# csukuangfj/kaldi-hmm-gmm

Measured on AMD Instinct MI355X. Metric: frames/sec (whole node) per EM iter (align+acc-stats), 5k-pdf x 64-Gauss, higher is better.
Workload: dtype f32 via f16x2s

## Files before the change

kaldi_hmm_gmm_amd/csrc/khg_k3.hip:

```cpp
#include "khg_internal.hpp"

#include <hipcub/hipcub.hpp>

#include "khg_k3_accstats.hip.inc"
#include "khg_k3_post.hip.inc"
#include "khg_k3_accops.hip.inc"

extern "C" int khg_accs_create(khg_ctx* ctx, const khg_model* m, const khg_tm* tm, khg_accs** out) {
  if (ctx_dead(ctx) || !m || !tm || !out) return khg_set_error(KHG_E_ARG, "khg_accs_create: bad arguments");
  khg_accs* a = new khg_accs();
  a->ctx = ctx; a->sumG = m->sumG; a->D = m->D; a->num_tids = tm->num_tids;
  a->n = a->sumG * (1 + 2 * (int64_t)a->D) + a->num_tids + 1 + 8;
  int rc = dev_alloc(&a->buf_d, (size_t)a->n);
  if (rc) { delete a; return rc; }
  a->cap = a->n;
  *out = a;
  return khg_accs_zero(ctx, a);
}
extern "C" int khg_accs_destroy(khg_accs* a) { if (a) { DEVFREE(a->buf_d); DEVFREE(a->wire_d); delete a; } return KHG_OK; }
extern "C" int khg_accs_zero(khg_ctx* ctx, khg_accs* a) {
  if (ctx_dead(ctx) || !a) return khg_set_error(KHG_E_ARG, "bad arguments");
  HIPCHK(hipMemsetAsync(a->buf_d, 0, sizeof(double) * (size_t)a->n, ctx->stream));
  return KHG_OK;
}
// ... 211 lines not shown
          KHG_LAUNCH(ctx, k3_sub_scan, dim3(1), dim3(1024), 0, ctx->stream, u->unc_d, u->frame_off_d, u->n_utt, u->sub_off_d);
          KHG_LAUNCH(ctx, k3_sub_keys, dim3((unsigned)std::min(u->n_utt, 8192)), dim3(64), 0, ctx->stream, a, u->unc_d, u->frame_off_d, u->sub_off_d, u->n_utt, sort_keys, sort_vals);
        } else if (tm->num_tids <= K3_LDS_TIDS) KHG_LAUNCH(ctx, k3_sort_keys<true>, dim3(std::min(gb, 1024)), dim3(256), 0, ctx->stream, a, sort_keys, sort_vals);
        else KHG_LAUNCH(ctx, k3_sort_keys<false>, dim3(std::min(gb, 1024)), dim3(256), 0, ctx->stream, a, sort_keys, sort_vals);
        HIPCHK(hipcub::DeviceRadixSort::SortPairs(sort_tmp, need, sort_keys, sort_keys_out, sort_vals,
                                                  reinterpret_cast<uint32_t*>(a.frame_ids), (int)Neff, 0, bits, ctx->stream));
        if (post) {
          K3Args b = a;
          b.num_tids = -1;
          KHG_LAUNCH(ctx, k3_bounds, dim3((m->P + 256) / 256), dim3(256), 0, ctx->stream, b, sort_keys_out);
        } else KHG_LAUNCH(ctx, k3_bounds, dim3((m->P + 256) / 256), dim3(256), 0, ctx->stream, a, sort_keys_out);
      }
    }
    int64_t k3_extra_blocks = 0;
    auto make_items = [&](int ny_base, bool parked, size_t nsum1, int cls_lo, int cls_hi, bool second) -> int {
      const int64_t avg = Neff / std::max(1, m->P);
      const int target = ctx->k3_one_block ? INT_MAX : (int)std::min<int64_t>(1 << 30, std::max<int64_t>(512, 2 * avg / ny_base));
      const int64_t per_t = Neff / target;
      k3_extra_blocks = std::min<int64_t>(per_t + m->P, 2 * per_t) + 1;
      const int64_t max_items = (int64_t)m->P * ny_base + k3_extra_blocks;
      const int64_t max_slots = !parked ? INT_MAX : ny_base > 1 ? max_items : 2 * per_t + 1;
      if (max_items >= INT_MAX / 2) return khg_set_error(KHG_E_UNSUPPORTED, "khg_acc_stats: too many work items");
      if (u->k3_items_n < (size_t)max_items) {
        DEVFREE(u->k3_items_d);
        { int ri = u_alloc(u, reinterpret_cast<K3Item**>(&u->k3_items_d), 2 * (size_t)max_items); if (ri) return ri; }
        u->k3_items_n = (size_t)max_items;
      }
      if (u->k3_item_off_n < (size_t)m->P + 1) {
        DEVFREE(u->k3_item_off_d);
        int rc2 = u_alloc(u, &u->k3_item_off_d, 2 * ((size_t)m->P + 1));
        if (rc2) return rc2;
        u->k3_item_off_n = (size_t)m->P + 1;
      }
      if (parked && u->k3_part_n < (size_t)max_slots * nsum1) {
        DEVFREE(u->k3_part_d);
        int rc2 = u_alloc(u, &u->k3_part_d, (size_t)max_slots * nsum1);
        if (rc2) return rc2;
        u->k3_part_n = (size_t)max_slots * nsum1;
      }
      K3Item* items = reinterpret_cast<K3Item*>(u->k3_items_d) + (second ? u->k3_items_n : 0);
      int32_t* item_off = u->k3_item_off_d + (second ? u->k3_item_off_n : 0);
      KHG_LAUNCH(ctx, k3_make_items, dim3(1), dim3(1024), 0, ctx->stream, a, ny_base, target, (int)max_items, (int)std::min<int64_t>(max_slots, INT_MAX),
                         items, item_off, cls_lo, cls_hi);
      a.items = items; a.item_off = item_off;
      return KHG_OK;
    };
    const int k3form = ctx->opt[KHG_OPT_K3_FORM];
    auto run_wave = [&](int cls_lo, int cls_hi, int maxG, void* comm_) -> int {
      const int nb = (maxG + 15) / 16;
      bool f16a = false;
      if (nb >= 3 && ctx->opt[KHG_OPT_K3_PHASE_A] == 0 && ctx->opt[KHG_OPT_K3_PHASE_B] != 1) { rc = k3_phase_a_scales(ctx, const_cast<khg_model*>(m), u, &f16a); if (rc) return rc; }
      if (f16a) {
        a.pa_ex = m->k3_ex_d; a.pa_S = m->k3_S;
        a.pa_scale = std::ldexp(1.0f, m->k3_S); a.pa_inv = std::ldexp(1.0f, -m->k3_S); a.pa_c1 = std::ldexp(1.44269504088896340736f, -m->k3_S);
      }
      const bool f16b = f16a && ctx->opt[KHG_OPT_K3_PHASE_B] == 2 && std::isfinite(weight) && std::fabs(weight) > 1.0e-30f && std::fabs(weight) < 1.0e30f;
      if (f16b) { a.pb_SG = 13 - std::ilogb(std::fabs(weight)); a.pb_gscale = std::ldexp(1.0f, a.pb_SG); }
      const size_t lds = std::max<size_t>(f16a ? sizeof(float) * (4 * 4 * 16 * 20) + 2 * (size_t)(4 * 2 * 16 * K3_XH_ROW)
                                               : sizeof(float) * ((size_t)nb * 20 * 64 + 4 * 4 * 16 * 20),
                                          sizeof(double) * ((size_t)nb * 16 * 80 + (size_t)nb * 16));
      const int64_t avg_tiles = (Neff / std::max(1, m->P) + 15) / 16;
      int ny = (int)std::max<int64_t>(1, std::min<int64_t>(std::min<int64_t>(32, (avg_tiles + 15) / 16), (4096 + m->P - 1) / m->P));
      if (ctx->opt[KHG_OPT_K3_NY] > 0) ny = ctx->opt[KHG_OPT_K3_NY];
      const size_t nsum1 = (size_t)nb * 16 * 80 + (size_t)nb * 16 + 1;
      if (u->k3_llpart_n < (size_t)m->P) {
        DEVFREE(u->k3_llpart_d);
        rc = u_alloc(u, &u->k3_llpart_d, (size_t)m->P);
        if (rc) return rc;
        u->k3_llpart_n = (size_t)m->P;
      }
      rc = make_items(ny, true, nsum1, cls_lo, cls_hi, false);
      if (rc) return rc;
      HIPCHK(hipMemsetAsync(u->k3_llpart_d, 0, sizeof(double) * (size_t)m->P, ctx->stream));
      a.ll_part = u->k3_llpart_d;
      a.part = u->k3_part_d;
      const int nparts_ = comm_ ? nparts : 1;
      for (int part = 0; part < nparts_; ++part) {
      const int p0 = (int)((int64_t)m->P * part / nparts_), np = (int)((int64_t)m->P * (part + 1) / nparts_) - p0;
      a.pdf0 = p0; a.npdf = np;
      const unsigned nblk = (unsigned)((int64_t)np * ny + k3_extra_blocks);
      {
      KernelTimer kt(ctx, nsub < 0 ? "k3_accumulate" : "k3_accumulate_pass2");
      const bool exact_b = true;
      const size_t lds16 = std::max<size_t>(2 * (size_t)4 * (2 * (2 * 16 * K3_XH_ROW) + 2 * 2 * 40 * 36) + (size_t)nb * 3 * 2 * 64 * 16,
                                            sizeof(double) * ((size_t)nb * 16 * 80 + (size_t)nb * 16));
#define K3_WAVE_LAUNCH(NBV)                                                                                            \
  do {                                                                                                                  \
    if (f16b) {                                                                                                          \
      HIPCHK(hipFuncSetAttribute((const void*)k3_accumulate_wave16<NBV>, hipFuncAttributeMaxDynamicSharedMemorySize, (int)lds16)); \
      KHG_LAUNCH(ctx, (k3_accumulate_wave16<NBV>), dim3(nblk), dim3(256), lds16, ctx->stream, a);                     \
    } else if (exact_b && f16a) KHG_LAUNCH(ctx, (k3_accumulate_wave<NBV, true>), dim3(nblk), dim3(256), lds, ctx->stream, a);    \
    else KHG_LAUNCH(ctx, (k3_accumulate_wave<NBV>), dim3(nblk), dim3(256), lds, ctx->stream, a);                      \
    KHG_LAUNCH(ctx, (k3_wave_finalize<NBV>), dim3(np), dim3(256), 0, ctx->stream, a);                                 \
  } while (0)
      switch (nb) {
        case 1: K3_WAVE_LAUNCH(1); break;
        case 2: K3_WAVE_LAUNCH(2); break;
        case 3: K3_WAVE_LAUNCH(3); break;
        default: K3_WAVE_LAUNCH(4); break;
      }
#undef K3_WAVE_LAUNCH
      }
      if (comm_ && nparts_ > 1) { rc = accs_allreduce_pieces(ctx, acc, m, p0, np, comm_, nullptr); if (rc) return rc; }
      }
      a.pdf0 = 0; a.npdf = m->P;
      KHG_LAUNCH(ctx, k3_wave_scalars, dim3(1), dim3(1024), 0, ctx->stream, a, cls_lo, cls_hi);
      return KHG_OK;
    };
    auto run_mfma = [&](int cls_lo, int cls_hi, int maxG, int n_cls, bool second, void* comm_) -> int {
      const int64_t avg_chunks = (Neff / std::max(1, m->P) + K3_CHUNK - 1) / K3_CHUNK;
      const size_t lds = sizeof(float) * ((size_t)4 * K3_CHUNK * 2 * m->KQ + (post ? 6 : 5) * K3_CHUNK);
      int ny = (int)std::max<int64_t>(1, std::min<int64_t>(std::min<int64_t>(32, avg_chunks), (4096 + n_cls - 1) / std::max(1, n_cls)));
      if (ctx->opt[KHG_OPT_K3_NY] > 0) ny = ctx->opt[KHG_OPT_K3_NY];
      if (ctx->k3_one_block) ny = 1;
      rc = make_items(ny, false, 0, cls_lo, cls_hi, second);
      if (rc) return rc;
      bool b16 = false;
      if (!post && ctx->opt[KHG_OPT_K3_PHASE_A] == 0 && ctx->opt[KHG_OPT_K3_PHASE_B] == 2 && ((m->KQ == 20 && maxG <= 128) || (m->KQ == 10 && maxG <= 192)) &&
          std::isfinite(weight) && std::fabs(weight) > 1.0e-30f && std::fabs(weight) < 1.0e30f) {
        rc = k3_phase_a_scales(ctx, const_cast<khg_model*>(m), u, &b16);
        if (rc) return rc;
      }
      if (b16) {
        a.pa_ex = m->k3_ex_d; a.pa_S = m->k3_S;
        a.pa_scale = std::ldexp(1.0f, m->k3_S); a.pa_inv = std::ldexp(1.0f, -m->k3_S); a.pa_c1 = std::ldexp(1.44269504088896340736f, -m->k3_S);
        a.pb_SG = 13 - std::ilogb(std::fabs(weight)); a.pb_gscale = std::ldexp(1.0f, a.pb_SG);
      }
      const size_t kpad = ((size_t)8 * m->KQ + 31) / 32 * 32;
      const size_t gp_b16 = maxG <= 64 ? 64 : (maxG <= 128 ? 128 : 192);
      const size_t lds_b16 = std::max<size_t>(2 * (2 * (size_t)K3_CHUNK * (kpad + 8) + 2 * (size_t)8 * m->KQ * (K3_CHUNK + 8)) + sizeof(float) * 9 * K3_CHUNK,
                                              sizeof(float) * (2 * gp_b16 * (size_t)(m->D | 1) + 8 * (size_t)m->KQ));
      const int nparts_ = comm_ ? nparts : 1;
      for (int part = 0; part < nparts_; ++part) {
        const int p0 = (int)((int64_t)m->P * part / nparts_), np = (int)((int64_t)m->P * (part + 1) / nparts_) - p0;
        a.pdf0 = p0; a.npdf = np;
        const unsigned nblk = (unsigned)((int64_t)std::min(np, n_cls) * ny + k3_extra_blocks);
        {
          KernelTimer kt(ctx, nsub < 0 ? "k3_accumulate" : "k3_accumulate_pass2");
          if (b16) {
#define K3_B16(KQV, NBWV, NWVV)                                                                                                 \
  do {                                                                                                                          \
    HIPCHK(hipFuncSetAttribute((const void*)k3_accumulate_block16<KQV, NBWV, NWVV>, hipFuncAttributeMaxDynamicSharedMemorySize, (int)lds_b16)); \
    KHG_LAUNCH(ctx, (k3_accumulate_block16<KQV, NBWV, NWVV>), dim3(nblk), dim3(64 * NWVV), lds_b16, ctx->stream, a);            \
  } while (0)
            if (maxG <= 64) { if (m->KQ == 20) K3_B16(20, 1, 4); else K3_B16(10, 1, 4); }
            else if (maxG <= 128) { if (m->KQ == 20) K3_B16(20, 1, 8); else K3_B16(10, 1, 8); }
            else K3_B16(10, 3, 4);
#undef K3_B16
          } else if (post) {
            if (m->KQ == 10 && maxG <= 64) KHG_LAUNCH(ctx, (k3_accumulate_mfma<10, 1, true>), dim3(nblk), dim3(256), lds, ctx->stream, a);
            else if (m->KQ == 10 && maxG <= 128) KHG_LAUNCH(ctx, (k3_accumulate_mfma<10, 2, true>), dim3(nblk), dim3(256), lds, ctx->stream, a);
            else if (m->KQ == 10 && maxG <= 192) KHG_LAUNCH(ctx, (k3_accumulate_mfma<10, 3, true>), dim3(nblk), dim3(256), lds, ctx->stream, a);
            else if (m->KQ == 10) KHG_LAUNCH(ctx, (k3_accumulate_mfma<10, 4, true>), dim3(nblk), dim3(256), lds, ctx->stream, a);
            else if (maxG <= 64) KHG_LAUNCH(ctx, (k3_accumulate_mfma<20, 1, true>), dim3(nblk), dim3(256), lds, ctx->stream, a);
            else KHG_LAUNCH(ctx, (k3_accumulate_mfma<20, 2, true>), dim3(nblk), dim3(256), lds, ctx->stream, a);
          } else
          if (m->KQ == 10 && maxG <= 64) KHG_LAUNCH(ctx, (k3_accumulate_mfma<10, 1>), dim3(nblk), dim3(256), lds, ctx->stream, a);
          else if (m->KQ == 10 && maxG <= 128) KHG_LAUNCH(ctx, (k3_accumulate_mfma<10, 2>), dim3(nblk), dim3(256), lds, ctx->stream, a);
          else if (m->KQ == 10 && maxG <= 192) KHG_LAUNCH(ctx, (k3_accumulate_mfma<10, 3>), dim3(nblk), dim3(256), lds, ctx->stream, a);
          else if (m->KQ == 10) KHG_LAUNCH(ctx, (k3_accumulate_mfma<10, 4>), dim3(nblk), dim3(256), lds, ctx->stream, a);
          else if (maxG <= 64) KHG_LAUNCH(ctx, (k3_accumulate_mfma<20, 1>), dim3(nblk), dim3(256), lds, ctx->stream, a);
          else KHG_LAUNCH(ctx, (k3_accumulate_mfma<20, 2>), dim3(nblk), dim3(256), lds, ctx->stream, a);
        }
        if (comm_ && nparts_ > 1) { rc = accs_allreduce_pieces(ctx, acc, m, p0, np, comm_, nullptr); if (rc) return rc; }
      }
      a.pdf0 = 0; a.npdf = m->P;
      return KHG_OK;
// ... 154 lines not shown
```

kaldi_hmm_gmm_amd/csrc/khg_k3_accstats.hip.inc:

```

struct K3Args {
  const float* feats;
  const int32_t* ali;
  const int32_t* id2pdf;
  int32_t num_tids;
  int64_t N;
  int32_t P, D;
  const int32_t* gauss_off;
  const float* gconsts;
  const float* means_invvars;
  const float* inv_vars;
  const float* nhalf_inv_vars;
  int32_t* pdf_count;
  int64_t* pdf_start;
  int32_t* pdf_cursor;
  int32_t* frame_ids;
  unsigned long long* tid_count;
  double* occ; double* mean_acc; double* var_acc; double* trans_acc; double* scalars;
  float weight;
  int32_t* err_flag;
  double* part;
  double* ll_part;
  int32_t pdf0, npdf;
  const struct K3Item* items;
// ... 797 lines not shown
          if (!(fabsf(llf) <= 3.0e38f)) atomicOr(a.err_flag, 1);
          tot_ll += (double)(llf * wf);
          if constexpr (POST) tot_w += (double)wf;
        }
        const float scale = f < cf ? wf / ssum : 0.0f;
#pragma unroll
        for (int k = 0; k < NBW; ++k) ll[k][ft][r] = ll[k][ft][r] * scale;
      }
#pragma unroll
    for (int ft = 0; ft < 4; ++ft) {
#pragma unroll
      for (int s = 0; s < 4; ++s) {
        const int fr = 16 * ft + 4 * q + s;
        double ga[NBW];
#pragma unroll
        for (int k = 0; k < NBW; ++k) { ga[k] = (double)ll[k][ft][s]; occ[k] += ga[k]; }
#pragma unroll
        for (int db = 0; db < NDB; ++db) {
          const int col = 16 * db + j16;
          const int d = col < XP ? col : col - XP;
          const double bv = (double)xq[(((col < XP ? 0 : 2) + (d & 1)) * K3_CHUNK + fr) * KH + (d >> 1)];
#pragma unroll
          for (int k = 0; k < NBW; ++k)
            acc[k][db] = __builtin_amdgcn_mfma_f64_16x16x4f64(ga[k], bv, acc[k][db], 0, 0, 0);
        }
      }
    }
  }
#pragma unroll
  for (int k = 0; k < NBW; ++k) {
    const int gb = 16 * (wave + 4 * k);
#pragma unroll
    for (int db = 0; db < NDB; ++db) {
      const int col = 16 * db + j16;
#pragma unroll
      for (int r = 0; r < 4; ++r) {
        const int g = gb + q + 4 * r;
        if (g < G) {
          if (col < D) atomicAdd(a.mean_acc + (int64_t)(g0 + g) * D + col, acc[k][db][r]);
          else if (col >= XP && col - XP < D) atomicAdd(a.var_acc + (int64_t)(g0 + g) * D + (col - XP), acc[k][db][r]);
        }
      }
    }
    double o = occ[k];
    o += __shfl_xor(o, 16);
    o += __shfl_xor(o, 32);
    if (q == 0 && gb + j16 < G) atomicAdd(a.occ + g0 + gb + j16, o);
  }
  if (wave == 0) {
    for (int o2 = 32; o2 > 0; o2 >>= 1) tot_ll += __shfl_xor(tot_ll, o2);
    if (lane == 0 && tot_ll != 0.0) atomicAdd(&a.scalars[1], tot_ll);
  }
  if constexpr (POST) {
    if (wave == 0) {
      for (int o2 = 32; o2 > 0; o2 >>= 1) tot_w += __shfl_xor(tot_w, o2);
      if (lane == 0 && tot_w != 0.0) atomicAdd(&a.scalars[0], tot_w);
    }
  } else {
    if (tid == 0 && it.y == 0) atomicAdd(&a.scalars[0], (double)nfr * (double)a.weight);
  }
}

typedef _Float16 k3_f16x8 __attribute__((ext_vector_type(8)));
#define K3_XH_ROW 104

template <int NB>
__device__ __forceinline__ void k3_wave_flush(const K3Args& a, const double* sum, int g0, int G, int D, int tid) {
  constexpr int XP = 40;
  for (int i = tid; i < NB * 16 * 2 * XP; i += 256) {
    const int g = i / (2 * XP), col = i - g * (2 * XP);
    if (g < G) {
      if (col < D) atomicAdd(a.mean_acc + (int64_t)(g0 + g) * D + col, sum[i]);
      else if (col >= XP && col - XP < D) atomicAdd(a.var_acc + (int64_t)(g0 + g) * D + (col - XP), sum[i]);
    }
  }
  if (tid < NB * 16 && tid < G) atomicAdd(a.occ + g0 + tid, sum[NB * 16 * 2 * XP + tid]);
}

__device__ __forceinline__ void k3_lds_sync() {
  asm volatile("s_waitcnt lgkmcnt(0)" ::: "memory");
  __builtin_amdgcn_wave_barrier();
}

template <int NB, bool F16A = false>
__global__ __launch_bounds__(256, NB <= 2 ? 2 : 1) void k3_accumulate_wave(K3Args a) {
  extern __shared__ __attribute__((aligned(16))) float k3s[];
  constexpr int KQ = 10, XP = 4 * KQ, KH = 2 * KQ, NDB = KQ / 2, TF = 16;
  K3Item it;
  if (!k3_take_item(a, it)) return;
  const int pdf = it.pdf;
  const int64_t beg = a.pdf_start[pdf];
  const int nfr = (int)(a.pdf_start[pdf + 1] - beg);
  if (nfr == 0) return;
  const int D = a.D;
  const int g0 = a.gauss_off[pdf], G = a.gauss_off[pdf + 1] - g0;
  const int tid = threadIdx.x, lane = tid & 63;
  const int wave = __builtin_amdgcn_readfirstlane(tid >> 6);
  const int j16 = lane & 15, q = lane >> 4;
  float* Wl = k3s;
  float* xw = (F16A ? k3s : Wl + NB * KH * 64) + wave * (4 * TF * KH);
  _Float16* xh = reinterpret_cast<_Float16*>(k3s + 4 * (4 * TF * KH)) + wave * (2 * TF * K3_XH_ROW);
  float gcv[NB];
#pragma unroll
  for (int k = 0; k < NB; ++k) gcv[k] = (16 * k + j16 < G) ? a.gconsts[g0 + 16 * k + j16] : -INFINITY;
  float wq[F16A ? 1 : NB][F16A ? 1 : KH];
  k3_f16x8 w1[F16A ? NB : 1][3], w2[F16A ? NB : 1][3];
  if constexpr (!F16A) {
    for (int idx = tid; idx < NB * KH * 64; idx += 256) {
      const int l = idx & 63, s = (idx >> 6) % KH, k = idx / (64 * KH);
      const int g = 16 * k + (l & 15), qq = l >> 4, d = 2 * s + (qq & 1);
      float v = 0.0f;
      if (g < G && d < D) v = (qq & 2) ? a.nhalf_inv_vars[(int64_t)(g0 + g) * D + d] : a.means_invvars[(int64_t)(g0 + g) * D + d];
      Wl[idx] = v;
    }
    __syncthreads();
#pragma unroll
    for (int k = 0; k < NB; ++k)
#pragma unroll
      for (int s = 0; s < KH; ++s) wq[k][s] = Wl[(k * KH + s) * 64 + lane];
  } else {
#pragma unroll
    for (int k = 0; k < NB; ++k)
#pragma unroll
      for (int st = 0; st < 3; ++st) {
        k3_f16x8 p1, p2;
#pragma unroll
        for (int e = 0; e < 8; ++e) {
          const int kp = 32 * st + 8 * q + e, var = kp >= XP, d = var ? kp - XP : kp, g = 16 * k + j16;
          float v = 0.0f;
          if (kp < 2 * XP && g < G && d < D) {
            const float w = var ? a.nhalf_inv_vars[(int64_t)(g0 + g) * D + d] : a.means_invvars[(int64_t)(g0 + g) * D + d];
            v = ldexpf(w, a.pa_S - a.pa_ex[2 * d + var]);
          }
          const _Float16 h1 = (_Float16)v;
          p1[e] = h1; p2[e] = (_Float16)(v - (float)h1);
        }
        w1[k][st] = p1; w2[k][st] = p2;
      }
#pragma unroll
    for (int k = 0; k < NB; ++k) gcv[k] = gcv[k] * a.pa_scale;
    for (int i = lane; i < 2 * TF * K3_XH_ROW; i += 64) xh[i] = (_Float16)0.0f;
    k3_lds_sync();
  }
  (void)Wl; (void)wq; (void)w1; (void)w2;

  f64x4 acc[NB][NDB];
  double occ[NB];
#pragma unroll
  for (int k = 0; k < NB; ++k) {
    occ[k] = 0.0;
#pragma unroll
    for (int db = 0; db < NDB; ++db) acc[k][db] = f64x4{0, 0, 0, 0};
  }
  double tot_ll = 0.0;
  const int ntile = (nfr + TF - 1) / TF;
  constexpr int NG = TF * XP / 64;
  const int tstride = 4 * it.ny;
  float pre[NG];
  float sx[F16A ? NG : 1], sx2[F16A ? NG : 1];
  if constexpr (F16A) {
#pragma unroll
    for (int j = 0; j < NG; ++j) {
      const int d = min((lane + 64 * j) % XP, D - 1);
      sx[j] = ldexpf(1.0f, a.pa_ex[2 * d]); sx2[j] = ldexpf(1.0f, a.pa_ex[2 * d + 1]);
    }
  }
// ... 70 lines not shown
      }
    }
#pragma unroll
    for (int r = 0; r < 4; ++r) {
      float m = ll[0][r];
#pragma unroll
      for (int k = 1; k < NB; ++k) m = fmaxf(m, ll[k][r]);
      m = k3_row_max(m);
      float ssum = 0.0f;
#pragma unroll
      for (int k = 0; k < NB; ++k) {
        const float e = __builtin_amdgcn_exp2f((ll[k][r] - m) * (F16A ? a.pa_c1 : 1.44269504088896340736f));
        ll[k][r] = e;
        ssum += e;
      }
      ssum = k3_row_sum(ssum);
      const int f = 4 * q + r;
      if (j16 == 0 && f < cf) {
        const float llf = __logf(ssum) + (F16A ? m * a.pa_inv : m);
        if (!(fabsf(llf) <= 3.0e38f)) atomicOr(a.err_flag, 1);
        tot_ll += (double)(llf * a.weight);
      }
      const float scale = f < cf ? a.weight / ssum : 0.0f;
#pragma unroll
      for (int k = 0; k < NB; ++k) ll[k][r] = ll[k][r] * scale;
    }
#pragma unroll
    for (int s = 0; s < 4; ++s) {
      const int fr = 4 * q + s;
      double ga[NB];
#pragma unroll
      for (int k = 0; k < NB; ++k) { ga[k] = (double)ll[k][s]; occ[k] += ga[k]; }
#pragma unroll
      for (int db = 0; db < NDB; ++db) {
        const int col = 16 * db + j16;
        const int d = col < XP ? col : col - XP;
        const double bv = (double)xw[(((col < XP ? 0 : 2) + (d & 1)) * TF + fr) * KH + (d >> 1)];
#pragma unroll
        for (int k = 0; k < NB; ++k)
          acc[k][db] = __builtin_amdgcn_mfma_f64_16x16x4f64(ga[k], bv, acc[k][db], 0, 0, 0);
      }
    }
    k3_lds_sync();
  }
  __syncthreads();
  double* sum = reinterpret_cast<double*>(k3s);
  constexpr int NSUM = NB * 16 * 2 * XP + NB * 16;
  for (int i = tid; i < NSUM; i += 256) sum[i] = 0.0;
  __syncthreads();
#pragma unroll 1
  for (int w = 0; w < 4; ++w) {
    if (wave == w) {
#pragma unroll
      for (int k = 0; k < NB; ++k) {
#pragma unroll
        for (int db = 0; db < NDB; ++db) {
          const int col = 16 * db + j16;
#pragma unroll
          for (int r = 0; r < 4; ++r) atomicAdd(&sum[(16 * k + q + 4 * r) * (2 * XP) + col], acc[k][db][r]);
        }
        double o = occ[k];
        o += __shfl_xor(o, 16);
        o += __shfl_xor(o, 32);
        if (q == 0) atomicAdd(&sum[NB * 16 * 2 * XP + 16 * k + j16], o);
      }
    }
    __syncthreads();
  }
  __shared__ double s_ll[4];
  for (int o2 = 32; o2 > 0; o2 >>= 1) tot_ll += __shfl_xor(tot_ll, o2);
  if (lane == 0) s_ll[wave] = tot_ll;
  __syncthreads();
  const double block_ll = ((s_ll[0] + s_ll[1]) + s_ll[2]) + s_ll[3];
  if (it.ny == 1) {
    k3_wave_flush<NB>(a, sum, g0, G, D, tid);
    if (tid == 0) a.ll_part[pdf] = block_ll;
  } else {
    double* dst = a.part + (int64_t)it.slot * (NSUM + 1);
    for (int i = tid; i < NSUM; i += 256) dst[i] = sum[i];
    if (tid == 0) dst[NSUM] = block_ll;
  }
}

template <int NB>
__global__ __launch_bounds__(256, 1) void k3_accumulate_wave16(K3Args a) {
  extern __shared__ __attribute__((aligned(16))) float k3s[];
  constexpr int KQ = 10, XP = 4 * KQ, NDB = KQ / 2, TF = 16;
  constexpr int XHH = 2 * TF * K3_XH_ROW;
  constexpr int XTR = 36, XTH = 2 * 2 * XP * XTR;
  K3Item it;
  if (!k3_take_item(a, it)) return;
  const int pdf = it.pdf;
  const int64_t beg = a.pdf_start[pdf];
  const int nfr = (int)(a.pdf_start[pdf + 1] - beg);
  if (nfr == 0) return;
  const int D = a.D;
  const int g0 = a.gauss_off[pdf], G = a.gauss_off[pdf + 1] - g0;
  const int tid = threadIdx.x, lane = tid & 63;
  const int wave = __builtin_amdgcn_readfirstlane(tid >> 6);
  const int j16 = lane & 15, q = lane >> 4;
  _Float16* xh = reinterpret_cast<_Float16*>(k3s) + wave * (2 * XHH + XTH);
  _Float16* xt = xh + 2 * XHH;
  float gcv[NB];
#pragma unroll
  for (int k = 0; k < NB; ++k) gcv[k] = ((16 * k + j16 < G) ? a.gconsts[g0 + 16 * k + j16] : -INFINITY) * a.pa_scale;
  char* wl16 = reinterpret_cast<char*>(reinterpret_cast<_Float16*>(k3s) + 4 * (2 * XHH + XTH));
  for (int e0 = tid; e0 < NB * 3 * 64; e0 += 256) {
    const int l = e0 & 63, st = (e0 >> 6) % 3, k = e0 / (3 * 64), jl = l & 15, ql = l >> 4;
    k3_f16x8 p1, p2;
#pragma unroll
    for (int e = 0; e < 8; ++e) {
      const int kp = 32 * st + 8 * ql + e, var = kp >= XP, d = var ? kp - XP : kp, g = 16 * k + jl;
      float v = 0.0f;
      if (kp < 2 * XP && g < G && d < D) {
        const float w = var ? a.nhalf_inv_vars[(int64_t)(g0 + g) * D + d] : a.means_invvars[(int64_t)(g0 + g) * D + d];
        v = ldexpf(w, a.pa_S - a.pa_ex[2 * d + var]);
      }
      const _Float16 h1 = (_Float16)v;
      p1[e] = h1; p2[e] = (_Float16)(v - (float)h1);
    }
    *reinterpret_cast<k3_f16x8*>(wl16 + (((k * 3 + st) * 2 + 0) * 64 + l) * 16) = p1;
    *reinterpret_cast<k3_f16x8*>(wl16 + (((k * 3 + st) * 2 + 1) * 64 + l) * 16) = p2;
  }
  {
    static_assert((2 * XHH + XTH) % 8 == 0, "the wave's planes are whole 16-byte words");
    const k3_f16x8 z = {0, 0, 0, 0, 0, 0, 0, 0};
    for (int i = lane; i < (2 * XHH + XTH) / 8; i += 64) reinterpret_cast<k3_f16x8*>(xh)[i] = z;
  }
  __syncthreads();

  f64x4 acc[NB][NDB];
  double occ[NB];
#pragma unroll
  for (int k = 0; k < NB; ++k) {
    occ[k] = 0.0;
#pragma unroll
    for (int db = 0; db < NDB; ++db) acc[k][db] = f64x4{0, 0, 0, 0};
  }
  double tot_ll = 0.0;
  unsigned bad = 0;
  const int ntile = (nfr + TF - 1) / TF, npair = (ntile + 1) / 2;
  constexpr int NM = 2 * TF * XP / (4 * 64);
  static_assert(NM * 4 * 64 == 2 * TF * XP, "micro-tiles cover the pair exactly");
  const int pstride = 4 * it.ny;
  float pre[NM][4];
  float sx[NM][2], sx2[NM][2];
  const bool even_d = (D & 1) == 0;
#pragma unroll
  for (int j = 0; j < NM; ++j)
#pragma unroll
    for (int c = 0; c < 2; ++c) {
      const int d = min(2 * ((lane + 64 * j) % 20) + c, D - 1);
      sx[j][c] = ldexpf(1.0f, a.pa_ex[2 * d]); sx2[j][c] = ldexpf(1.0f, a.pa_ex[2 * d + 1]);
    }
  const float gs = a.pb_gscale;
  const int rot = (int)(((unsigned)pdf * 2654435761u) % (unsigned)npair);
  auto pair_of = [&](int p) { const int x = p + rot; return x >= npair ? x - npair : x; };
  auto cf_of = [&](int pl, int tau) { if (pl >= npair) return 0; const int t = 2 * pair_of(pl) + tau; return t < ntile ? min(TF, nfr - t * TF) : 0; };
  auto fid_of = [&](int pl, int tau) -> int {
    const int n = cf_of(pl, tau);
    const int t = pl < npair ? 2 * pair_of(pl) + tau : 0;
    return lane < n ? a.frame_ids[beg + t * TF + lane] : 0;
  };
  auto request = [&](int fid0, int fid1) {
    int fa[NM], fb[NM];
#pragma unroll
    for (int j = 0; j < NM; ++j) {
      const int i = lane + 64 * j, tau = i / 160, fp = (i % 160) / 20;
      if (j < 2) { fa[j] = __shfl(fid0, 2 * fp); fb[j] = __shfl(fid0, 2 * fp + 1); }
      else if (j > 2) { fa[j] = __shfl(fid1, 2 * fp); fb[j] = __shfl(fid1, 2 * fp + 1); }
      else {
        const int a0 = __shfl(fid0, 2 * fp), a1 = __shfl(fid1, 2 * fp), b0 = __shfl(fid0, 2 * fp + 1), b1 = __shfl(fid1, 2 * fp + 1);
        fa[j] = tau ? a1 : a0; fb[j] = tau ? b1 : b0;
      }
    }
#pragma unroll
    for (int j = 0; j < NM; ++j) {
      const int d0 = 2 * ((lane + 64 * j) % 20);
      if (even_d) {
        typedef float f2 __attribute__((ext_vector_type(2)));
        const int dd = min(d0, D - 2);
        const f2 va = *reinterpret_cast<const f2*>(a.feats + (int64_t)fa[j] * D + dd), vb = *reinterpret_cast<const f2*>(a.feats + (int64_t)fb[j] * D + dd);
        pre[j][0] = va[0]; pre[j][1] = va[1]; pre[j][2] = vb[0]; pre[j][3] = vb[1];
      } else {
        const int da = min(d0, D - 1), db = min(d0 + 1, D - 1);
        pre[j][0] = a.feats[(int64_t)fa[j] * D + da]; pre[j][1] = a.feats[(int64_t)fa[j] * D + db];
        pre[j][2] = a.feats[(int64_t)fb[j] * D + da]; pre[j][3] = a.feats[(int64_t)fb[j] * D + db];
      }
    }
  };
  int p = it.y * 4 + wave;
  int fidn0 = 0, fidn1 = 0;
  if (p < npair) { request(fid_of(p, 0), fid_of(p, 1)); fidn0 = fid_of(p + pstride, 0); fidn1 = fid_of(p + pstride, 1); }
  for (; p < npair; p += pstride) {
    const int cf[2] = {cf_of(p, 0), cf_of(p, 1)};
#pragma unroll
    for (int j = 0; j < NM; ++j) {
      typedef _Float16 h2v __attribute__((ext_vector_type(2)));
      const int i = lane + 64 * j, tau = i / 160, r = i % 160, f0 = 2 * (r / 20), d0 = 2 * (r % 20);
      const int cft = tau ? cf[1] : cf[0];
      _Float16 h1[4], h2[4], g1[4], g2[4];
#pragma unroll
      for (int e = 0; e < 4; ++e) {
        const int f = f0 + (e >> 1), d = d0 + (e & 1);
        const float v = (f < cft && d < D) ? pre[j][e] : 0.0f;
        const float s1 = v * sx[j][e & 1], s2 = (v * v) * sx2[j][e & 1];
        h1[e] = (_Float16)s1; g1[e] = (_Float16)s2;
        h2[e] = (_Float16)(s1 - (float)h1[e]); g2[e] = (_Float16)(s2 - (float)g1[e]);
      }
#pragma unroll
      for (int ff = 0; ff < 2; ++ff) {
        _Float16* r1 = xh + tau * XHH + (f0 + ff) * K3_XH_ROW + d0;
        *reinterpret_cast<h2v*>(r1) = h2v{h1[2 * ff], h1[2 * ff + 1]};
        *reinterpret_cast<h2v*>(r1 + TF * K3_XH_ROW) = h2v{h2[2 * ff], h2[2 * ff + 1]};
        *reinterpret_cast<h2v*>(r1 + XP) = h2v{g1[2 * ff], g1[2 * ff + 1]};
        *reinterpret_cast<h2v*>(r1 + TF * K3_XH_ROW + XP) = h2v{g2[2 * ff], g2[2 * ff + 1]};
      }
#pragma unroll
      for (int dd = 0; dd < 2; ++dd) {
        _Float16* c1 = xt + (d0 + dd) * XTR + tau * TF + f0;
        *reinterpret_cast<h2v*>(c1) = h2v{h1[dd], h1[2 + dd]};
        *reinterpret_cast<h2v*>(c1 + 2 * XP * XTR) = h2v{h2[dd], h2[2 + dd]};
        *reinterpret_cast<h2v*>(c1 + XP * XTR) = h2v{g1[dd], g1[2 + dd]};
        *reinterpret_cast<h2v*>(c1 + 2 * XP * XTR + XP * XTR) = h2v{g2[dd], g2[2 + dd]};
      }
    }
    if (p + pstride < npair) { request(fidn0, fidn1); fidn0 = fid_of(p + 2 * pstride, 0); fidn1 = fid_of(p + 2 * pstride, 1); }
    k3_lds_sync();
    f32x4 ll[2][NB];
#pragma unroll
    for (int tau = 0; tau < 2; ++tau)
#pragma unroll
      for (int k = 0; k < NB; ++k) ll[tau][k] = f32x4{gcv[k], gcv[k], gcv[k], gcv[k]};
#pragma unroll
    for (int st = 0; st < 3; ++st) {
      k3_f16x8 x1[2], x2[2];
#pragma unroll
      for (int tau = 0; tau < 2; ++tau) {
        x1[tau] = *reinterpret_cast<const k3_f16x8*>(xh + tau * XHH + j16 * K3_XH_ROW + 32 * st + 8 * q);
        x2[tau] = *reinterpret_cast<const k3_f16x8*>(xh + tau * XHH + (TF + j16) * K3_XH_ROW + 32 * st + 8 * q);
      }
#pragma unroll
      for (int k = 0; k < NB; ++k) {
        const k3_f16x8 wa = *reinterpret_cast<const k3_f16x8*>(wl16 + (((k * 3 + st) * 2 + 0) * 64 + lane) * 16);
        const k3_f16x8 wb = *reinterpret_cast<const k3_f16x8*>(wl16 + (((k * 3 + st) * 2 + 1) * 64 + lane) * 16);
#pragma unroll
        for (int tau = 0; tau < 2; ++tau) {
          ll[tau][k] = __builtin_amdgcn_mfma_f32_16x16x32_f16(x2[tau], wa, ll[tau][k], 0, 0, 0);
          ll[tau][k] = __builtin_amdgcn_mfma_f32_16x16x32_f16(x1[tau], wb, ll[tau][k], 0, 0, 0);
          ll[tau][k] = __builtin_amdgcn_mfma_f32_16x16x32_f16(x1[tau], wa, ll[tau][k], 0, 0, 0);
        }
      }
    }
#pragma unroll
    for (int tau = 0; tau < 2; ++tau) {
#pragma unroll
      for (int r = 0; r < 4; ++r) {
        float m = ll[tau][0][r];
#pragma unroll
        for (int k = 1; k < NB; ++k) m = fmaxf(m, ll[tau][k][r]);
        m = k3_row_max(m);
        float ssum = 0.0f;
#pragma unroll
        for (int k = 0; k < NB; ++k) {
          const float e = __builtin_amdgcn_exp2f((ll[tau][k][r] - m) * a.pa_c1);
          ll[tau][k][r] = e;
          ssum += e;
        }
        ssum = k3_row_sum(ssum);
        const int f = 4 * q + r;
        const bool counts = (j16 == 0) & (f < cf[tau]);
        const float llf = __logf(ssum) + m * a.pa_inv;
        bad |= (counts & !(fabsf(llf) <= 3.0e38f)) ? 1u : 0u;
        tot_ll += counts ? (double)(llf * a.weight) : 0.0;
        const float scale = f < cf[tau] ? a.weight / ssum : 0.0f;
#pragma unroll
        for (int k = 0; k < NB; ++k) ll[tau][k][r] = ll[tau][k][r] * scale;
      }
    }
    k3_f16x8 ga1[NB], ga2[NB];
    f32x4 prev[NB];
#pragma unroll
    for (int k = 0; k < NB; ++k) {
#pragma unroll
      for (int e = 0; e < 8; ++e) {
        const float g = e < 4 ? ll[0][k][e] : ll[1][k][e - 4];
        occ[k] += (double)g;
        const float gsc = g * gs;
        const _Float16 h1 = (_Float16)gsc;
        ga1[k][e] = h1; ga2[k][e] = (_Float16)(gsc - (float)h1);
      }
    }
#pragma unroll
    for (int db = 0; db < NDB; ++db) {
      const _Float16* cb = xt + (16 * db + j16) * XTR + 4 * q;
      k3_f16x8 xb1, xb2;
      {
        typedef _Float16 h4 __attribute__((ext_vector_type(4)));
        const h4 a0 = *reinterpret_cast<const h4*>(cb), a1 = *reinterpret_cast<const h4*>(cb + TF);
        const h4 b0 = *reinterpret_cast<const h4*>(cb + 2 * XP * XTR), b1 = *reinterpret_cast<const h4*>(cb + 2 * XP * XTR + TF);
#pragma unroll
        for (int e = 0; e < 4; ++e) { xb1[e] = a0[e]; xb1[4 + e] = a1[e]; xb2[e] = b0[e]; xb2[4 + e] = b1[e]; }
      }
      f32x4 cur[NB];
#pragma unroll
      for (int k = 0; k < NB; ++k) {
        f32x4 c = f32x4{0, 0, 0, 0};
        c = __builtin_amdgcn_mfma_f32_16x16x32_f16(ga1[k], xb2, c, 0, 0, 0);
        c = __builtin_amdgcn_mfma_f32_16x16x32_f16(ga2[k], xb1, c, 0, 0, 0);
        c = __builtin_amdgcn_mfma_f32_16x16x32_f16(ga1[k], xb1, c, 0, 0, 0);
        cur[k] = c;
      }
      if (db > 0) {
#pragma unroll
        for (int k = 0; k < NB; ++k)
#pragma unroll
          for (int r = 0; r < 4; ++r) acc[k][db - 1][r] += (double)prev[k][r];
      }
#pragma unroll
      for (int k = 0; k < NB; ++k) prev[k] = cur[k];
    }
#pragma unroll
    for (int k = 0; k < NB; ++k)
#pragma unroll
      for (int r = 0; r < 4; ++r) acc[k][NDB - 1][r] += (double)prev[k][r];
    k3_lds_sync();
  }
  __syncthreads();
  double* sum = reinterpret_cast<double*>(k3s);
  constexpr int NSUM = NB * 16 * 2 * XP + NB * 16;
  for (int i = tid; i < NSUM; i += 256) sum[i] = 0.0;
  __syncthreads();
  int unscale[NDB];
#pragma unroll
  for (int db = 0; db < NDB; ++db) {
    const int col = 16 * db + j16, var = col >= XP, d = min(var ? col - XP : col, D - 1);
    unscale[db] = -(a.pb_SG + a.pa_ex[2 * d + var]);
  }
#pragma unroll 1
  for (int ph = 0; ph < 4; ++ph) {
    const int kk = (wave + ph) & 3;
#pragma unroll
    for (int k = 0; k < NB; ++k) {
      if (k != kk) continue;
#pragma unroll
      for (int db = 0; db < NDB; ++db) {
        const int col = 16 * db + j16;
#pragma unroll
        for (int r = 0; r < 4; ++r) atomicAdd(&sum[(16 * k + 4 * q + r) * (2 * XP) + col], ldexp(acc[k][db][r], unscale[db]));
      }
      double o = occ[k];
      o += __shfl_xor(o, 16);
      o += __shfl_xor(o, 32);
      if (q == 0) atomicAdd(&sum[NB * 16 * 2 * XP + 16 * k + j16], o);
    }
    __syncthreads();
  }
  if (bad) atomicOr(a.err_flag, 1);
  __shared__ double s_ll[4];
  for (int o2 = 32; o2 > 0; o2 >>= 1) tot_ll += __shfl_xor(tot_ll, o2);
  if (lane == 0) s_ll[wave] = tot_ll;
  __syncthreads();
  const double block_ll = ((s_ll[0] + s_ll[1]) + s_ll[2]) + s_ll[3];
  if (it.ny == 1) {
    k3_wave_flush<NB>(a, sum, g0, G, D, tid);
    if (tid == 0) a.ll_part[pdf] = block_ll;
  } else {
    double* dst = a.part + (int64_t)it.slot * (NSUM + 1);
    for (int i = tid; i < NSUM; i += 256) dst[i] = sum[i];
    if (tid == 0) dst[NSUM] = block_ll;
  }
}

#ifndef K3B16_KO
#define K3B16_KO 0
#endif
template <int KQ, int NBW, int NWV>
__global__ __launch_bounds__(64 * NWV, 1) void k3_accumulate_block16(K3Args a) {
  constexpr int NT = 64 * NWV;
  extern __shared__ __attribute__((aligned(16))) float k3s[];
  constexpr int XP = 4 * KQ;
  constexpr int K2 = 2 * XP;
  constexpr int KPAD = (K2 + 31) / 32 * 32, KST = KPAD / 32;
  constexpr int NDB = K2 / 16;
  constexpr int XROW = KPAD + 8;
  constexpr int XTR = K3_CHUNK + 8;
  constexpr int XHH = K3_CHUNK * XROW, XTH = K2 * XTR;
  static_assert((XROW / 8) % 2 == 1 && (XTR / 8) % 2 == 1, "row pitches are odd multiples of 16 bytes");
  K3Item it;
  if (!k3_take_item(a, it)) return;
  const int pdf = it.pdf;
  const int64_t beg = a.pdf_start[pdf];
  const int nfr = (int)(a.pdf_start[pdf + 1] - beg);
  if (nfr == 0) return;
  const int D = a.D;
  const int g0 = a.gauss_off[pdf], G = a.gauss_off[pdf + 1] - g0;
  _Float16* xh = reinterpret_cast<_Float16*>(k3s);
  _Float16* xt = xh + 2 * XHH;
  float* red = reinterpret_cast<float*>(xt + 2 * XTH);
  float* fin = red + NWV * K3_CHUNK;
  const int tid = threadIdx.x, lane = tid & 63;
  const int wave = __builtin_amdgcn_readfirstlane(tid >> 6);
  const int j16 = lane & 15, q = lane >> 4;
  const int nchunk = (nfr + K3_CHUNK - 1) / K3_CHUNK;

  constexpr int GP = 16 * NBW * NWV;
  k3_f16x8 w1[NBW][KST], w2[NBW][KST];
  float gcv[NBW];
  {
    const int WP = D | 1;
    float* wl = k3s;
    int* ewl = reinterpret_cast<int*>(wl + 2 * GP * WP);
    for (int idx = tid; idx < G * D; idx += NT) {
      const int g = idx / D, d = idx - g * D;
      float mi = 0.0f, nh = 0.0f;
      if (!(K3B16_KO & 64)) { mi = a.means_invvars[(int64_t)g0 * D + idx]; nh = a.nhalf_inv_vars[(int64_t)g0 * D + idx]; }
      wl[g * WP + d] = mi; wl[(GP + g) * WP + d] = nh;
    }
    for (int kp = tid; kp < K2; kp += NT) {
      const int var = kp >= XP, d = var ? kp - XP : kp;
      ewl[kp] = d < D ? a.pa_S - a.pa_ex[2 * d + var] : 0;
    }
    k3_block_sync();
#pragma unroll
    for (int k = 0; k < NBW; ++k) {
      const int g = 16 * (wave + NWV * k) + j16;
      const bool gv = g < G;
      gcv[k] = (gv ? a.gconsts[g0 + g] : -INFINITY) * a.pa_scale;
#pragma unroll
      for (int st = 0; st < KST; ++st) {
#pragma unroll
        for (int e = 0; e < 8; ++e) {
          const int kp = 32 * st + 8 * q + e, var = kp >= XP, d = var ? kp - XP : kp;
          float v = 0.0f;
          if (kp < K2 && gv && d < D) v = ldexpf(wl[(var * GP + g) * WP + d], ewl[kp]);
          const _Float16 h1 = (_Float16)v;
          w1[k][st][e] = h1; w2[k][st][e] = (_Float16)(v - (float)h1);
        }
      }
// ... 302 lines not shown
```

Baseline: 441.0 million.

## Accumulate MFMA results in fp32 across tiles and use transposed LDS reads

The f16 accumulate kernel no longer writes a separate transposed copy of each feature tile into LDS. It reads the row-major planes directly with ds_read_tr16 transpose loads. MFMA results now accumulate in fp32 registers across several tiles and are periodically exchanged through LDS, where each wave owns one Gaussian block and folds the partials into fp64 totals. This replaces per-tile fp64 conversion and the final LDS atomic reduction with plain stores, shrinking LDS per wave, at the cost of extra block-wide barriers and longer fp32 accumulation chains.

```diff
diff --git a/kaldi_hmm_gmm_amd/csrc/khg_k3.hip b/kaldi_hmm_gmm_amd/csrc/khg_k3.hip
--- a/kaldi_hmm_gmm_amd/csrc/khg_k3.hip
+++ b/kaldi_hmm_gmm_amd/csrc/khg_k3.hip
@@ -317,7 +317,7 @@
       {
       KernelTimer kt(ctx, nsub < 0 ? "k3_accumulate" : "k3_accumulate_pass2");
       const bool exact_b = true;
-      const size_t lds16 = std::max<size_t>(2 * (size_t)4 * (2 * (2 * 16 * K3_XH_ROW) + 2 * 2 * 40 * 36) + (size_t)nb * 3 * 2 * 64 * 16,
+      const size_t lds16 = std::max<size_t>((size_t)4 * K3W16_AREA + (size_t)nb * 3 * 2 * 64 * 16,
                                             sizeof(double) * ((size_t)nb * 16 * 80 + (size_t)nb * 16));
 #define K3_WAVE_LAUNCH(NBV)                                                                                            \
   do {                                                                                                                  \
diff --git a/kaldi_hmm_gmm_amd/csrc/khg_k3_accstats.hip.inc b/kaldi_hmm_gmm_amd/csrc/khg_k3_accstats.hip.inc
--- a/kaldi_hmm_gmm_amd/csrc/khg_k3_accstats.hip.inc
+++ b/kaldi_hmm_gmm_amd/csrc/khg_k3_accstats.hip.inc
@@ -903,6 +903,15 @@
   __builtin_amdgcn_wave_barrier();
 }
 
+typedef _Float16 k3_f16x4 __attribute__((ext_vector_type(4)));
+__device__ __forceinline__ k3_f16x4 k3_lds_read_tr16(const _Float16* p) {
+  typedef short s4 __attribute__((__vector_size__(4 * sizeof(short))));
+  const s4 v = __builtin_amdgcn_ds_read_tr16_b64_v4i16((__attribute__((address_space(3))) s4*)(p));
+  k3_f16x4 r;
+  __builtin_memcpy(&r, &v, sizeof(r));
+  return r;
+}
+
 template <int NB, bool F16A = false>
 __global__ __launch_bounds__(256, NB <= 2 ? 2 : 1) void k3_accumulate_wave(K3Args a) {
   extern __shared__ __attribute__((aligned(16))) float k3s[];
@@ -1139,12 +1148,15 @@
   }
 }
 
+#define K3W16_R 4
+#define K3W16_AREA 20992
 template <int NB>
 __global__ __launch_bounds__(256, 1) void k3_accumulate_wave16(K3Args a) {
   extern __shared__ __attribute__((aligned(16))) float k3s[];
   constexpr int KQ = 10, XP = 4 * KQ, NDB = KQ / 2, TF = 16;
   constexpr int XHH = 2 * TF * K3_XH_ROW;
-  constexpr int XTR = 36, XTH = 2 * 2 * XP * XTR;
+  constexpr int XOCC = 4 * NDB * 64 * 16, WAREA = K3W16_AREA;
+  static_assert(2 * 2 * XHH <= WAREA && XOCC + 4 * 16 * 8 <= WAREA && WAREA % 16 == 0, "planes and exchange fit a wave's area");
   K3Item it;
   if (!k3_take_item(a, it)) return;
   const int pdf = it.pdf;
@@ -1156,12 +1168,11 @@
   const int tid = threadIdx.x, lane = tid & 63;
   const int wave = __builtin_amdgcn_readfirstlane(tid >> 6);
   const int j16 = lane & 15, q = lane >> 4;
-  _Float16* xh = reinterpret_cast<_Float16*>(k3s) + wave * (2 * XHH + XTH);
-  _Float16* xt = xh + 2 * XHH;
+  _Float16* xh = reinterpret_cast<_Float16*>(reinterpret_cast<char*>(k3s) + wave * WAREA);
   float gcv[NB];
 #pragma unroll
   for (int k = 0; k < NB; ++k) gcv[k] = ((16 * k + j16 < G) ? a.gconsts[g0 + 16 * k + j16] : -INFINITY) * a.pa_scale;
-  char* wl16 = reinterpret_cast<char*>(reinterpret_cast<_Float16*>(k3s) + 4 * (2 * XHH + XTH));
+  char* wl16 = reinterpret_cast<char*>(k3s) + 4 * WAREA;
   for (int e0 = tid; e0 < NB * 3 * 64; e0 += 256) {
     const int l = e0 & 63, st = (e0 >> 6) % 3, k = e0 / (3 * 64), jl = l & 15, ql = l >> 4;
     k3_f16x8 p1, p2;
@@ -1180,20 +1191,24 @@
     *reinterpret_cast<k3_f16x8*>(wl16 + (((k * 3 + st) * 2 + 1) * 64 + l) * 16) = p2;
   }
   {
-    static_assert((2 * XHH + XTH) % 8 == 0, "the wave's planes are whole 16-byte words");
+    static_assert((2 * XHH) % 8 == 0, "the wave's planes are whole 16-byte words");
     const k3_f16x8 z = {0, 0, 0, 0, 0, 0, 0, 0};
-    for (int i = lane; i < (2 * XHH + XTH) / 8; i += 64) reinterpret_cast<k3_f16x8*>(xh)[i] = z;
-  }
-  __syncthreads();
-
-  f64x4 acc[NB][NDB];
+    for (int i = lane; i < (2 * XHH) / 8; i += 64) reinterpret_cast<k3_f16x8*>(xh)[i] = z;
+  }
+  __syncthreads();
+
+  f32x4 part[NB][NDB];
+  f64x4 tot[NDB];
   double occ[NB];
+#pragma unroll
+  for (int db = 0; db < NDB; ++db) tot[db] = f64x4{0, 0, 0, 0};
 #pragma unroll
   for (int k = 0; k < NB; ++k) {
     occ[k] = 0.0;
 #pragma unroll
-    for (int db = 0; db < NDB; ++db) acc[k][db] = f64x4{0, 0, 0, 0};
-  }
+    for (int db = 0; db < NDB; ++db) part[k][db] = f32x4{0, 0, 0, 0};
+  }
+  double occ_own = 0.0;
   double tot_ll = 0.0;
   unsigned bad = 0;
   const int ntile = (nfr + TF - 1) / TF, npair = (ntile + 1) / 2;
@@ -1246,10 +1261,56 @@
       }
     }
   };
+  char* const xbase = reinterpret_cast<char*>(k3s);
+  auto exchange = [&](const bool last) {
+    char* const mine = xbase + wave * WAREA;
+#pragma unroll
+    for (int k = 0; k < NB; ++k) {
+#pragma unroll
+      for (int db = 0; db < NDB; ++db) *reinterpret_cast<f32x4*>(mine + ((k * NDB + db) * 64 + lane) * 16) = part[k][db];
+      if (last) {
+        double o = occ[k];
+        o += __shfl_xor(o, 16);
+        o += __shfl_xor(o, 32);
+        if (q == 0) reinterpret_cast<double*>(mine + XOCC)[16 * k + j16] = o;
+      }
+    }
+#pragma unroll
+    for (int k = 0; k < NB; ++k)
+#pragma unroll
+      for (int db = 0; db < NDB; ++db) part[k][db] = f32x4{0, 0, 0, 0};
+    __syncthreads();
+    if (wave < NB) {
+#pragma unroll
+      for (int v = 0; v < 4; ++v) {
+#pragma unroll
+        for (int db = 0; db < NDB; ++db) {
+          const f32x4 pv = *reinterpret_cast<const f32x4*>(xbase + v * WAREA + ((wave * NDB + db) * 64 + lane) * 16);
+#pragma unroll
+          for (int r = 0; r < 4; ++r) tot[db][r] += (double)pv[r];
+        }
+      }
+      if (last) {
+        double o = 0.0;
+#pragma unroll
+        for (int i = 0; i < 4; ++i) o += reinterpret_cast<const double*>(xbase + ((wave + 4 - i) & 3) * WAREA + XOCC)[16 * wave + j16];
+        occ_own = o;
+      }
+    }
+    __syncthreads();
+    if (!last) {
+      const k3_f16x8 z = {0, 0, 0, 0, 0, 0, 0, 0};
+#pragma unroll
+      for (int i = lane; i < 2 * 2 * TF * 2; i += 64) *reinterpret_cast<k3_f16x8*>(xh + (i >> 1) * K3_XH_ROW + 2 * XP + 8 * (i & 1)) = z;
+    }
+  };
+  const int niter = npair > it.y * 4 ? (npair - it.y * 4 + pstride - 1) / pstride : 0;
   int p = it.y * 4 + wave;
   int fidn0 = 0, fidn1 = 0;
   if (p < npair) { request(fid_of(p, 0), fid_of(p, 1)); fidn0 = fid_of(p + pstride, 0); fidn1 = fid_of(p + pstride, 1); }
-  for (; p < npair; p += pstride) {
+#pragma unroll 1
+  for (int iter = 0; iter < niter; ++iter, p += pstride) {
+    if (p < npair) {
     const int cf[2] = {cf_of(p, 0), cf_of(p, 1)};
 #pragma unroll
     for (int j = 0; j < NM; ++j) {
@@ -1272,14 +1333,6 @@
         *reinterpret_cast<h2v*>(r1 + TF * K3_XH_ROW) = h2v{h2[2 * ff], h2[2 * ff + 1]};
         *reinterpret_cast<h2v*>(r1 + XP) = h2v{g1[2 * ff], g1[2 * ff + 1]};
         *reinterpret_cast<h2v*>(r1 + TF * K3_XH_ROW + XP) = h2v{g2[2 * ff], g2[2 * ff + 1]};
-      }
-#pragma unroll
-      for (int dd = 0; dd < 2; ++dd) {
-        _Float16* c1 = xt + (d0 + dd) * XTR + tau * TF + f0;
-        *reinterpret_cast<h2v*>(c1) = h2v{h1[dd], h1[2 + dd]};
-        *reinterpret_cast<h2v*>(c1 + 2 * XP * XTR) = h2v{h2[dd], h2[2 + dd]};
-        *reinterpret_cast<h2v*>(c1 + XP * XTR) = h2v{g1[dd], g1[2 + dd]};
-        *reinterpret_cast<h2v*>(c1 + 2 * XP * XTR + XP * XTR) = h2v{g2[dd], g2[2 + dd]};
       }
     }
     if (p + pstride < npair) { request(fidn0, fidn1); fidn0 = fid_of(p + 2 * pstride, 0); fidn1 = fid_of(p + 2 * pstride, 1); }
@@ -1336,7 +1389,6 @@
       }
     }
     k3_f16x8 ga1[NB], ga2[NB];
-    f32x4 prev[NB];
 #pragma unroll
     for (int k = 0; k < NB; ++k) {
 #pragma unroll
@@ -1350,68 +1402,38 @@
     }
 #pragma unroll
     for (int db = 0; db < NDB; ++db) {
-      const _Float16* cb = xt + (16 * db + j16) * XTR + 4 * q;
+      const _Float16* cb = xh + (4 * q + ((lane >> 2) & 3)) * K3_XH_ROW + 16 * db + 4 * (lane & 3);
       k3_f16x8 xb1, xb2;
       {
-        typedef _Float16 h4 __attribute__((ext_vector_type(4)));
-        const h4 a0 = *reinterpret_cast<const h4*>(cb), a1 = *reinterpret_cast<const h4*>(cb + TF);
-        const h4 b0 = *reinterpret_cast<const h4*>(cb + 2 * XP * XTR), b1 = *reinterpret_cast<const h4*>(cb + 2 * XP * XTR + TF);
+        const k3_f16x4 a0 = k3_lds_read_tr16(cb), a1 = k3_lds_read_tr16(cb + XHH);
+        const k3_f16x4 b0 = k3_lds_read_tr16(cb + TF * K3_XH_ROW), b1 = k3_lds_read_tr16(cb + XHH + TF * K3_XH_ROW);
 #pragma unroll
         for (int e = 0; e < 4; ++e) { xb1[e] = a0[e]; xb1[4 + e] = a1[e]; xb2[e] = b0[e]; xb2[4 + e] = b1[e]; }
       }
-      f32x4 cur[NB];
-#pragma unroll
-      for (int k = 0; k < NB; ++k) {
-        f32x4 c = f32x4{0, 0, 0, 0};
-        c = __builtin_amdgcn_mfma_f32_16x16x32_f16(ga1[k], xb2, c, 0, 0, 0);
-        c = __builtin_amdgcn_mfma_f32_16x16x32_f16(ga2[k], xb1, c, 0, 0, 0);
-        c = __builtin_amdgcn_mfma_f32_16x16x32_f16(ga1[k], xb1, c, 0, 0, 0);
-        cur[k] = c;
-      }
-      if (db > 0) {
-#pragma unroll
-        for (int k = 0; k < NB; ++k)
-#pragma unroll
-          for (int r = 0; r < 4; ++r) acc[k][db - 1][r] += (double)prev[k][r];
-      }
-#pragma unroll
-      for (int k = 0; k < NB; ++k) prev[k] = cur[k];
-    }
-#pragma unroll
-    for (int k = 0; k < NB; ++k)
-#pragma unroll
-      for (int r = 0; r < 4; ++r) acc[k][NDB - 1][r] += (double)prev[k][r];
+#pragma unroll
+      for (int k = 0; k < NB; ++k) part[k][db] = __builtin_amdgcn_mfma_f32_16x16x32_f16(ga1[k], xb2, part[k][db], 0, 0, 0);
+#pragma unroll
+      for (int k = 0; k < NB; ++k) part[k][db] = __builtin_amdgcn_mfma_f32_16x16x32_f16(ga2[k], xb1, part[k][db], 0, 0, 0);
+#pragma unroll
+      for (int k = 0; k < NB; ++k) part[k][db] = __builtin_amdgcn_mfma_f32_16x16x32_f16(ga1[k], xb1, part[k][db], 0, 0, 0);
+    }
     k3_lds_sync();
-  }
-  __syncthreads();
+    }
+    if ((iter + 1) % K3W16_R == 0 && iter + 1 < niter) exchange(false);
+  }
+  exchange(true);
   double* sum = reinterpret_cast<double*>(k3s);
   constexpr int NSUM = NB * 16 * 2 * XP + NB * 16;
-  for (int i = tid; i < NSUM; i += 256) sum[i] = 0.0;
-  __syncthreads();
-  int unscale[NDB];
-#pragma unroll
-  for (int db = 0; db < NDB; ++db) {
-    const int col = 16 * db + j16, var = col >= XP, d = min(var ? col - XP : col, D - 1);
-    unscale[db] = -(a.pb_SG + a.pa_ex[2 * d + var]);
-  }
-#pragma unroll 1
-  for (int ph = 0; ph < 4; ++ph) {
-    const int kk = (wave + ph) & 3;
-#pragma unroll
-    for (int k = 0; k < NB; ++k) {
-      if (k != kk) continue;
-#pragma unroll
-      for (int db = 0; db < NDB; ++db) {
-        const int col = 16 * db + j16;
-#pragma unroll
-        for (int r = 0; r < 4; ++r) atomicAdd(&sum[(16 * k + 4 * q + r) * (2 * XP) + col], ldexp(acc[k][db][r], unscale[db]));
-      }
-      double o = occ[k];
-      o += __shfl_xor(o, 16);
-      o += __shfl_xor(o, 32);
-      if (q == 0) atomicAdd(&sum[NB * 16 * 2 * XP + 16 * k + j16], o);
-    }
-    __syncthreads();
+  static_assert(NSUM * 8 <= 4 * WAREA, "the image fits the planes");
+  if (wave < NB) {
+#pragma unroll
+    for (int db = 0; db < NDB; ++db) {
+      const int col = 16 * db + j16, var = col >= XP, d = min(var ? col - XP : col, D - 1);
+      const int unscale = -(a.pb_SG + a.pa_ex[2 * d + var]);
+#pragma unroll
+      for (int r = 0; r < 4; ++r) sum[(16 * wave + 4 * q + r) * (2 * XP) + col] = ldexp(tot[db][r], unscale);
+    }
+    if (q == 0) sum[NB * 16 * 2 * XP + 16 * wave + j16] = occ_own;
   }
   if (bad) atomicOr(a.err_flag, 1);
   __shared__ double s_ll[4];
```

Measured after the change: 444.2 million, median of 6. No clear change (+0.7%).
